# jeongminpark417/COALA-GNN

Measured on AMD Instinct MI355X. Metric: feature-gather GB/s (payload = rows x dim x 4 B delivered per second), IGB-medium GraphSAGE minibatch fetch, higher is better.
Workload: dtype f32

## Files before the change

coala-gnn_amd/COALA_GNN_Pybind/__init__.py:

```python
import ctypes as C
import os
import sys

from . import _capi
from ._capi import CacheConfig, CacheGeometry, CacheProfile, check

_lib = _capi.load()

native = None
if os.path.realpath(_capi.LIB_PATH) == os.path.realpath(os.path.join(os.path.dirname(os.path.abspath(__file__)), os.pardir, "lib", "libcoala_hip.so")):
    try:
        from . import _coala_pybind as native
        if native.abi_version() != _lib.coala_abi_version():
            native = None
    except ImportError:
        native = None

__all__ = [
    "SharedUVAManager", "SSD_GNN_SSD_Controllers", "SSD_GNN_NVSHMEM_Cache", "Isolated_Cache", "Node_distributor_pybind",
    "NVSHMEM_Manager", "Graph_Coloring", "current_stream", "set_stream_provider", "native",
]


def _default_stream_provider():
# ... 150 lines not shown
        if node_distributer is not None:
            color_ptr = node_distributer.get_color_buffer_ptr()
            num_colors = node_distributer.get_num_colors()
            entries = node_distributer.get_num_color_entries()
        if num_rows is None:
            num_rows = entries
        if not num_rows:
            raise RuntimeError("number of feature rows unknown: pass num_rows= or a distributor built with a colour file")
        cfg.num_rows = int(num_rows)
        if color_ptr and entries and entries < cfg.num_rows:
            raise RuntimeError(f"colour table has {entries} entries but the feature table has {cfg.num_rows} rows")
        cfg.node_color = color_ptr
        cfg.num_colors = num_colors
        cfg.max_batch = int(max_batch)
        self._h = C.c_void_p()
        self.dim = ctrls.dim
        self.num_color = num_colors
        self.global_rank = int(g_rank)
        self.local_rank = int(rank)
        self.num_gpus = int(n_gpus)
        check(_lib.coala_cache_create(C.byref(cfg), C.byref(self._h)))
        self._keepalive = node_distributer

    def get_cache_data(self, ret_i_ptr, n_entries=None):
        n = self.num_color if n_entries is None else int(n_entries)
        check(_lib.coala_cache_color_counts(self._h, int(ret_i_ptr), n, current_stream()))

    def get_cache_data_async(self, n_entries=None):
        n = self.num_color if n_entries is None else int(n_entries)
        check(_lib.coala_cache_color_counts_async(self._h, n, current_stream()))

    def get_cache_data_finish(self, ret_i_ptr, n_entries=None):
        n = self.num_color if n_entries is None else int(n_entries)
        check(_lib.coala_cache_color_counts_finish(self._h, int(ret_i_ptr), n))

    def stats(self, reset=False):
        hit, miss, bad = C.c_uint64(), C.c_uint64(), C.c_uint64()
        check(_lib.coala_cache_stats(self._h, C.byref(hit), C.byref(miss), C.byref(bad), int(reset), current_stream()))
        return hit.value, miss.value, bad.value

    def print_stats(self):
        hit, miss, bad = self.stats(reset=True)
        print(f"Global Rank: {self.global_rank} Local Rank:{self.local_rank} hit count: {hit} miss count: {miss}")
        ratio = hit / (hit + miss) if hit + miss else float("nan")
        print(f"Global Rank: {self.global_rank} Local Rank:{self.local_rank}  GPU hit ratio: {ratio:f}")
        if bad:
            print(f"Global Rank: {self.global_rank} Local Rank:{self.local_rank} rejected ids: {bad}")

    def geometry(self):
        g = CacheGeometry()
        check(_lib.coala_cache_geometry(self._h, C.byref(g)))
        return g

    def profile(self, reset=False):
        p = CacheProfile()
        check(_lib.coala_cache_profile(self._h, C.byref(p), int(reset)))
        return p

    def fetch_events(self, enable=True):
        _capi.check(_lib.coala_cache_fetch_events(self._h, 1 if enable else 0))

    def last_fetch_events(self):
        a, b = C.c_void_p(), C.c_void_p()
        _capi.check(_lib.coala_cache_last_fetch_events(self._h, C.byref(a), C.byref(b)))
        return a.value, b.value

    def dump(self):
        import numpy as np
        g = self.geometry()
        keys = np.empty((g.num_sets, 32), dtype=np.uint64)
        cnt = np.empty(g.num_sets, dtype=np.uint32)
        meta = np.empty((g.num_sets, 32), dtype=np.uint32)
        check(_lib.coala_cache_dump(self._h, keys.ctypes.data, cnt.ctypes.data, meta.ctypes.data, current_stream()))
        return keys, cnt, meta

    def close(self):
        if getattr(self, "_h", None):
            _lib.coala_cache_destroy(self._h)
            self._h = C.c_void_p()

    def __del__(self):
        try:
            self.close()
        except Exception:
            pass

    def _read(self, out_ptr, idx_ptr, n):
        if native is not None:
            native.cache_read_feature(self._h.value or 0, int(out_ptr), int(idx_ptr), int(n), current_stream())
        else:
            check(_lib.coala_cache_read_feature(self._h, int(out_ptr), int(idx_ptr), int(n), current_stream()))

    def _serve(self, out_ptr, ids_ptr, n):
        if native is not None:
            native.cache_serve(self._h.value or 0, int(out_ptr), int(ids_ptr), int(n), current_stream())
        else:
            check(_lib.coala_cache_serve(self._h, int(out_ptr), int(ids_ptr), int(n), current_stream()))

    def serve_probe(self, out_ptr, ids_ptr, n):
        check(_lib.coala_cache_serve_probe(self._h, int(out_ptr), int(ids_ptr), int(n), current_stream()))

    def serve_fill(self, out_ptr, ids_ptr, n, begin, end):
        check(_lib.coala_cache_serve_fill(self._h, int(out_ptr), int(ids_ptr), int(n), int(begin), int(end), current_stream()))

    def serve_probe_redirect(self, out_ptr, ids_ptr, n, begin, end, redirect_out_ptr, row_map_ptr=0):
        rd = _capi.RowRedirect(int(begin), int(end), int(redirect_out_ptr) or None, int(row_map_ptr) or None)
# ... 159 lines not shown
```

coala-gnn_amd/COALA_GNN_Pybind/_capi.py:

```python
import ctypes as C
import os

_HERE = os.path.dirname(os.path.abspath(__file__))
LIB_PATH = os.environ.get("COALA_HIP_LIB", os.path.join(os.path.dirname(_HERE), "lib", "libcoala_hip.so"))

OK, EINVAL, EHIP, ENOMEM, EIO, EFORMAT, ERANGE, ECOMM = 0, -1, -2, -3, -4, -5, -6, -7
FLAG_SYNC, FLAG_DISTRIBUTED, FLAG_PROFILE, FLAG_COLD_PARTITIONED, FLAG_TAG64 = 1, 2, 4, 8, 16
WAYS = 32
COUNTS_RING = 8


class CacheConfig(C.Structure):
    _fields_ = [
        ("device", C.c_int32), ("dim", C.c_int32), ("cache_mb", C.c_uint64), ("n_gpus", C.c_int32), ("rank", C.c_int32),
        ("global_rank", C.c_int32), ("flags", C.c_uint32), ("cold_table", C.c_void_p), ("num_rows", C.c_uint64),
        ("node_color", C.c_void_p), ("num_colors", C.c_int32), ("reserved", C.c_int32), ("max_batch", C.c_uint64),
    ]


class CacheGeometry(C.Structure):
    _fields_ = [("num_sets", C.c_uint64), ("num_ways", C.c_uint32), ("cache_dim", C.c_uint32), ("line_bytes", C.c_uint64),
                ("table_bytes", C.c_uint64), ("tag_set_bytes", C.c_uint32), ("reserved", C.c_uint32)]


class CacheProfile(C.Structure):
    _fields_ = [("gather_ms", C.c_double), ("gather_launches", C.c_uint64), ("gather_rows", C.c_uint64),
                ("gather_hits", C.c_uint64), ("fill_ms", C.c_double), ("fill_launches", C.c_uint64),
                ("fill_rows", C.c_uint64), ("event_overhead_us", C.c_double)]


class RowRedirect(C.Structure):
    _fields_ = [("begin", C.c_int64), ("end", C.c_int64), ("out", C.c_void_p), ("row_map", C.c_void_p)]


class SamplerBucketing(C.Structure):
    _fields_ = [("n_parts", C.c_int32), ("reserved", C.c_int32), ("bucketed_nodes", C.c_void_p), ("counts", C.c_void_p),
                ("dst_in_src", C.c_void_p)]


class SamplerLayer(C.Structure):
    _fields_ = [("src_nodes", C.c_void_p), ("nbr_local", C.c_void_p), ("indptr_local", C.c_void_p), ("src_cap", C.c_int64),
                ("edge_cap", C.c_int64)]


class CommProfile(C.Structure):
    _fields_ = [("rows_ms", C.c_double), ("calls", C.c_uint64), ("remote_rows_in", C.c_uint64)]


_VP, _I, _I64, _U64, _SZ = C.c_void_p, C.c_int, C.c_int64, C.c_uint64, C.c_size_t
SYMBOLS = {
    "coala_last_error": (C.c_char_p, []),
    "coala_abi_version": (_I, []),
    "coala_cache_dim": (_I, [_I]),
    "coala_cache_num_sets": (_U64, [_U64, _I]),
    "coala_cache_create": (_I, [C.POINTER(CacheConfig), C.POINTER(_VP)]),
    "coala_cache_destroy": (_I, [_VP]),
    "coala_cache_geometry": (_I, [_VP, C.POINTER(CacheGeometry)]),
    "coala_cache_read_feature": (_I, [_VP, _VP, _VP, _I64, _VP]),
    "coala_cache_serve": (_I, [_VP, _VP, _VP, _I64, _VP]),
    "coala_cache_serve_probe": (_I, [_VP, _VP, _VP, _I64, _VP]),
    "coala_cache_serve_fill": (_I, [_VP, _VP, _VP, _I64, _I64, _I64, _VP]),
    "coala_cache_serve_fill_ranges": (_I, [_VP, _VP, _VP, _I64, C.POINTER(_I64), C.POINTER(_I64), _I, _VP]),
    "coala_cache_serve_abort": (_I, [_VP, _VP]),
    "coala_cache_serve_probe_redirect": (_I, [_VP, _VP, _VP, _I64, C.POINTER(RowRedirect), _VP]),
    "coala_cache_route": (_I, [_VP, _VP, _I64, _I, _I64, _VP, _VP, _VP, _VP, _VP]),
    "coala_cache_scatter": (_I, [_VP, _VP, _VP, _VP, _I64, _VP]),
    "coala_cache_scatter_ranges": (_I, [_VP, _VP, _VP, _VP, C.POINTER(_I64), C.POINTER(_I64), _I, _VP]),
    "coala_cache_row_dim": (_I64, [_VP]),
    "coala_cache_fetch_events": (_I, [_VP, _I]),
    "coala_cache_last_fetch_events": (_I, [_VP, C.POINTER(_VP), C.POINTER(_VP)]),
    "coala_stream_wait_event": (_I, [_VP, _VP]),
    "coala_event_elapsed_ms": (_I, [_VP, _VP, _I, C.POINTER(C.c_float)]),
    "coala_comm_unique_id": (_I, [_VP, _SZ]),
    "coala_comm_create": (_I, [_VP, _I, _I, _I, C.POINTER(_VP)]),
    "coala_comm_destroy": (_I, [_VP]),
    "coala_comm_size": (_I, [_VP]),
    "coala_comm_group_create": (_I, [_I, C.POINTER(_VP)]),
    "coala_comm_group_destroy": (_I, [_VP]),
    "coala_comm_create_inproc": (_I, [_VP, _I, _I, C.POINTER(_VP)]),
    "coala_comm_set_rounds": (_I, [_VP, _I]),
    "coala_comm_get_rounds": (_I, [_VP]),
    "coala_comm_set_self_loopback": (_I, [_VP, _I]),
    "coala_comm_fetch_events": (_I, [_VP, _I]),
    "coala_comm_last_fetch_events": (_I, [_VP, C.POINTER(_VP), C.POINTER(_VP), C.POINTER(_VP)]),
    "coala_comm_profile": (_I, [_VP, _I, C.POINTER(CommProfile), _I]),
    "coala_comm_last_counts": (_I, [_VP, _VP, _VP]),
    "coala_cache_fetch_distributed": (_I, [_VP, _VP, _VP, _VP, _I64, _VP]),
    "coala_cache_fetch_distributed_bucketed": (_I, [_VP, _VP, _VP, _VP, _I64, _VP, _VP]),
    "coala_comm_counts_begin": (_I, [_VP, _VP, _VP, _VP]),
    "coala_cache_fetch_distributed_bucketed_ahead": (_I, [_VP, _VP, _VP, _VP, _I64, _I64, _VP]),
    "coala_cache_color_counts": (_I, [_VP, _VP, C.c_int32, _VP]),
    "coala_cache_color_counts_async": (_I, [_VP, C.c_int32, _VP]),
    "coala_cache_color_counts_finish": (_I, [_VP, _VP, C.c_int32]),
    "coala_cache_stats": (_I, [_VP, C.POINTER(_U64), C.POINTER(_U64), C.POINTER(_U64), _I, _VP]),
    "coala_cache_dump": (_I, [_VP, _VP, _VP, _VP, _VP]),
    "coala_cache_profile": (_I, [_VP, C.POINTER(CacheProfile), _I]),
    "coala_coloring_create": (_I, [_U64, C.POINTER(_VP)]),
    "coala_coloring_destroy": (_I, [_VP]),
    "coala_coloring_set_adj_csc": (_I, [_VP, _VP, _VP]),
    "coala_coloring_set_color_buffer": (_I, [_VP, _VP]),
    "coala_coloring_set_topk_buffers": (_I, [_VP, _VP, _VP, _I]),
    "coala_coloring_color_optimized": (_I, [_VP, _VP, _U64, C.c_uint]),
    "coala_coloring_color_all": (_I, [_VP, C.c_uint]),
    "coala_coloring_num_color": (_U64, [_VP]),
    "coala_coloring_num_color_node": (_U64, [_VP]),
    "coala_coloring_topk": (_I, [_VP, _I]),
    "coala_coloring_nearest": (_I, [_VP]),
    "coala_sampler_create": (_I, [_I, _VP, _VP, _I64, _I64, C.POINTER(_VP)]),
    "coala_sampler_destroy": (_I, [_VP]),
    "coala_sampler_sample": (_I, [_VP, _VP, _I64, C.POINTER(C.c_int32), _I, _U64, _U64, C.POINTER(_VP), C.POINTER(_VP),
# ... 95 lines not shown
```

coala-gnn_amd/csrc/coala_cache.hip:

```cpp
#include <hip/hip_runtime.h>
#include <hip/hip_ext.h>

#include <algorithm>
#include <cstdarg>
#include <cstdio>
#include <cstdlib>
#include <cstring>
#include <new>
#include <type_traits>
#include <utility>
#include <vector>

#include "../../include/coala_hip.h"
#include "coala_internal.h"

namespace {

constexpr uint64_t kEmptyKey = 0xFFFFFFFFFFFFFFFFull;
constexpr uint32_t kLinkMiss = 0x80000000u;
constexpr uint32_t kLinkBad = 0x7FFFFFFFu;
constexpr int kStatBlocks = 2048;
constexpr int kFillSlots = 8;

struct CacheDev {
// ... 236 lines not shown
            const bool h = (G::RPP == 2 && sub) ? h_b : h_a;
            const V* src = reinterpret_cast<const V*>(c.lines + (uint64_t)s * CD);
#pragma unroll
            for (int v = 0; v < G::VPL; ++v) {
                const uint32_t u = v * G::LPR + l_in;
                if (h && (FULL || u < nunits)) val[p][v] = nt_load(src + u);
            }
        }
        if (!SINGLE) {
            tags = load_tags(ids_next);
            ids_next = ids_next2;
        }
#pragma unroll
        for (int p = 0; p < G::PASSES; ++p) {
            const int q = p * G::RPP + sub;
            const bool h_a = row_hit(p * G::RPP), h_b = row_hit(p * G::RPP + (G::RPP - 1));
            const bool bad_a = row_bad(p * G::RPP), bad_b2 = row_bad(p * G::RPP + (G::RPP - 1));
            const bool h = (G::RPP == 2 && sub) ? h_b : h_a;
            const bool bad = (G::RPP == 2 && sub) ? bad_b2 : bad_a;
            V* dst = reinterpret_cast<V*>(out + (base + q) * (int64_t)c.dim);
            if (REDIR) {
                auto row_drow = [&](int r) { return (int32_t)__builtin_amdgcn_readlane(drow_v[r / TG::SPL], TG::LPS * (r % TG::SPL)); };
                const int32_t dr_a = row_drow(p * G::RPP), dr_b = row_drow(p * G::RPP + (G::RPP - 1));
                const int32_t dr = (G::RPP == 2 && sub) ? dr_b : dr_a;
                if (dr >= 0) dst = reinterpret_cast<V*>(rd.out + (int64_t)dr * (int64_t)c.dim);
            }
#pragma unroll
            for (int v = 0; v < G::VPL; ++v) {
                const uint32_t u = v * G::LPR + l_in;
                if (FULL || u < nunits) {
                    if (h) dst[u] = val[p][v];
                    else if (bad) dst[u] = V(0.0f);
                }
            }
        }
#pragma unroll
        for (int t = 0; t < TSTEPS; ++t) {
            if (lead_l[t]) {
                uint32_t w = 0u;
                if (imiss_l[t]) w = kLinkMiss | (((uint32_t)(prev[t] >> 32) == gen) ? (uint32_t)prev[t] : 0u);
                else if (bad_l[t]) w = kLinkBad;
                c.miss_link[base + t * TG::SPL + lane / TG::LPS] = w;
            }
        }
        if (SINGLE) break;
    }
}

__device__ __forceinline__ uint64_t shfl64(uint64_t v, int src) {
    const uint32_t lo = __shfl((int)(uint32_t)v, src), hi = __shfl((int)(uint32_t)(v >> 32), src);
    return ((uint64_t)hi << 32) | lo;
}

template <int CD, int VEC, bool REDIR = false, int NP = 4>
__global__ __launch_bounds__(256) void miss_fill_kernel(CacheDev c, const int64_t* __restrict__ idx, float* __restrict__ out,
                                                        int tile_rows, int sparse_max, uint32_t gen, RangeSet rs, Redirect rd, int dyn_slot) {
    using G = Geo<CD, VEC, NP>;
    using V = typename VecT<VEC>::type;
    constexpr int R = G::R;
    const int lane = threadIdx.x & 63;
    const int64_t wave = (int64_t)blockIdx.x * (blockDim.x >> 6) + (threadIdx.x >> 6);
    const int64_t n_waves = (int64_t)gridDim.x * (blockDim.x >> 6);
    const int64_t n_tiles = ((int64_t)rs.total + tile_rows - 1) / tile_rows;
    const int chunks_per_tile = tile_rows / R;
    const uint32_t nunits = c.dim / VEC;
    const int sub = (G::RPP == 2) ? (lane >> 5) : 0;
    const int l_in = lane & (G::LPR - 1);
    uint32_t my_miss = 0, my_bad = 0;

    constexpr int U = 8;
    uint32_t* ticket = reinterpret_cast<uint32_t*>(c.stats + 2 * kStatBlocks) + (dyn_slot < 0 ? 0 : dyn_slot);
    const bool dyn = dyn_slot >= 0;
    if (reinterpret_cast<const uint32_t*>(c.stats + 2 * kStatBlocks)[2 * kFillSlots + (gen & 1u)] == 0u) return;
    const int64_t n_deal = dyn ? 1 : n_waves;
    const int64_t even8 = n_tiles / (n_waves * 8);
    const int claim_min = even8 < 1 ? 1 : (even8 > U ? U : (int)even8);
    int claim = claim_min;
    for (int64_t unit = dyn ? -1 : wave;;) {
      int64_t claim_end = n_tiles;
      if (dyn) {
          uint32_t t = 0;
          if (lane == 0) t = atomicAdd(ticket, (uint32_t)claim);
          unit = (int64_t)(uint32_t)__builtin_amdgcn_readfirstlane((int)t);
          if (unit >= n_tiles) break;
          claim_end = unit + claim < n_tiles ? unit + claim : n_tiles;
          claim = claim * 2 > 4 * U ? 4 * U : claim * 2;
      } else if (unit >= n_tiles) break;
     for (int64_t tile0 = unit; tile0 < claim_end; tile0 += n_deal * U) {
      const int n_here = dyn ? (int)(claim_end - tile0 < U ? claim_end - tile0 : U) : U;
      uint64_t st_pack = 0;
#pragma unroll
      for (int u = 0; u < U; ++u) {
          const int64_t tile = tile0 + u * n_deal;
          const uint32_t p = (u < n_here && tile < n_tiles && lane < tile_rows) ? pos_of(rs, (uint32_t)(tile * tile_rows + lane)) : 0xFFFFFFFFu;
          const uint32_t w = (p != 0xFFFFFFFFu) ? c.miss_link[p] : 0u;
          const uint64_t v = (w == 0u) ? 0u : ((w & kLinkMiss) ? 1u : 2u);
          st_pack |= v << (8 * u);
      }
      if (!__ballot(st_pack != 0)) continue;
      uint32_t slot_l = 0, win_l = 0;
      uint64_t id_l = 0;
      int64_t drow_l = 0;
      auto rank_at = [&](uint32_t pos) {
          id_l = (uint64_t)idx[pos];
          drow_l = (int64_t)pos;
          if (REDIR && (int64_t)pos >= rd.begin && (int64_t)pos < rd.end)
              drow_l = -((rd.row_map ? rd.row_map[(int64_t)pos - rd.begin] : (int64_t)pos - rd.begin) + 1);
          const uint64_t set = set_of(c, id_l);
          uint32_t cur = (uint32_t)c.set_head[set];
          uint32_t total = 0, rank = 0;
          while (cur) {
              const uint32_t p2 = cur - 1;
              ++total;
              rank += (p2 < pos) ? 1u : 0u;
              cur = c.miss_link[p2] & ~kLinkMiss;
          }
          const uint64_t cv = __hip_atomic_load(c.set_cnt + set, __ATOMIC_RELAXED, __HIP_MEMORY_SCOPE_AGENT);
          const uint32_t cnt0 = ((uint32_t)(cv >> 32) == gen) ? (uint32_t)cv - total : (uint32_t)cv;
          if (rank == 0) __hip_atomic_store(c.set_cnt + set, ((uint64_t)gen << 32) | (uint32_t)(cnt0 + total), __ATOMIC_RELAXED, __HIP_MEMORY_SCOPE_AGENT);
          const uint32_t way = (cnt0 + rank) & (COALA_WAYS - 1);
          slot_l = (uint32_t)(set * COALA_WAYS) + way;
          win_l = (rank + COALA_WAYS >= total) ? 1u : 0u;
          if (win_l) {
              if (c.tag32) reinterpret_cast<uint32_t*>(c.keys)[slot_l] = (uint32_t)id_l;
              else reinterpret_cast<uint64_t*>(c.keys)[slot_l] = id_l;
              if (c.color_counters) {
                  const int32_t col = c.node_color[id_l];
                  atomicSub(c.color_counters + c.color_meta[slot_l], 1);
                  atomicAdd(c.color_counters + col, 1);
                  c.color_meta[slot_l] = (uint32_t)col;
              }
          }
      };
      auto move_group = [&](const int (&srcl)[G::PASSES], const bool (&live)[G::PASSES]) {
          V val[G::PASSES][G::VPL];
          uint32_t slot_[G::PASSES];
          uint64_t id[G::PASSES];
          int64_t drow[G::PASSES];
          bool winner[G::PASSES];
#pragma unroll
          for (int p = 0; p < G::PASSES; ++p) {
              slot_[p] = (uint32_t)__shfl((int)slot_l, srcl[p]);
              winner[p] = __shfl((int)win_l, srcl[p]) != 0;
              id[p] = shfl64(id_l, srcl[p]);
              drow[p] = (int64_t)shfl64((uint64_t)drow_l, srcl[p]);
          }
#pragma unroll
          for (int p = 0; p < G::PASSES; ++p) {
              const V* src = reinterpret_cast<const V*>(c.cold + cold_row_of(c, id[p]) * (uint64_t)c.dim);
#pragma unroll
              for (int v = 0; v < G::VPL; ++v) {
                  const uint32_t u = v * G::LPR + l_in;
                  if (live[p] && u < nunits) val[p][v] = nt_load(src + u);
              }
          }
#pragma unroll
          for (int p = 0; p < G::PASSES; ++p) {
              V* dst = (REDIR && drow[p] < 0) ? reinterpret_cast<V*>(rd.out + (uint64_t)(-(drow[p] + 1)) * c.dim)
                                              : reinterpret_cast<V*>(out + (uint64_t)drow[p] * c.dim);
              V* line = reinterpret_cast<V*>(c.lines + (uint64_t)slot_[p] * CD);
#pragma unroll
              for (int v = 0; v < G::VPL; ++v) {
                  const uint32_t u = v * G::LPR + l_in;
                  if (live[p] && u < nunits) {
                      nt_store(val[p][v], dst + u);
                      if (winner[p]) nt_store(val[p][v], line + u);
                  }
              }
          }
      };
      auto stream_holders = [&](uint64_t holders) {
          int srcl[G::PASSES];
          bool live[G::PASSES];
          while (holders) {
#pragma unroll
              for (int p = 0; p < G::PASSES; ++p) {
                  int l0 = -1, l1 = -1;
                  if (holders) { l0 = __builtin_ctzll(holders); holders &= holders - 1; }
                  if (G::RPP == 2 && holders) { l1 = __builtin_ctzll(holders); holders &= holders - 1; }
                  const int l = (G::RPP == 2 && sub) ? l1 : l0;
                  live[p] = l >= 0;
                  srcl[p] = l >= 0 ? l : 0;
              }
              move_group(srcl, live);
          }
      };
      uint64_t mmask[U];
      uint32_t total_miss = 0, worst = 0;
#pragma unroll
      for (int u = 0; u < U; ++u) {
          const uint8_t st = (uint8_t)(st_pack >> (8 * u));
          mmask[u] = __ballot(st == 1);
          my_miss += (st == 1);
          my_bad += (st == 2);
          const uint32_t cnt = (uint32_t)__builtin_popcountll(mmask[u]);
          total_miss += cnt;
          worst = cnt > worst ? cnt : worst;
      }
      if (!total_miss) continue;
      claim = claim_min;
      if (total_miss <= 64 && (int)worst <= sparse_max) {
          uint32_t k = (uint32_t)lane;
          int u_sel = -1;
          uint64_t m_sel = 0;
#pragma unroll
          for (int u = 0; u < U; ++u) {
              const uint32_t cnt = (uint32_t)__builtin_popcountll(mmask[u]);
              if (u_sel < 0) {
                  if (k < cnt) { u_sel = u; m_sel = mmask[u]; }
                  else k -= cnt;
              }
          }
          if (u_sel >= 0) {
              for (uint32_t i = 0; i < k; ++i) m_sel &= m_sel - 1;
              const uint32_t pos = pos_of(rs, (uint32_t)((tile0 + u_sel * n_deal) * tile_rows + __builtin_ctzll(m_sel)));
              rank_at(pos);
          }
          stream_holders(total_miss >= 64 ? ~0ull : ((1ull << total_miss) - 1ull));
          continue;
      }
#pragma nounroll
      for (int u = 0; u < U; ++u) {
        const uint8_t st = (uint8_t)(st_pack >> (8 * u));
        const uint64_t tile_mask = __ballot(st == 1);
        if (!tile_mask) continue;
        const uint32_t pos_l = st ? pos_of(rs, (uint32_t)((tile0 + u * n_deal) * tile_rows + lane)) : 0u;
        if (__builtin_popcountll(tile_mask) <= sparse_max) {
            if (st == 1) rank_at(pos_l);
            stream_holders(tile_mask);
        } else {
            int srcl[G::PASSES];
            bool live[G::PASSES];
            for (int ck = 0; ck < chunks_per_tile; ++ck) {
                const uint32_t live_mask = (uint32_t)(tile_mask >> (ck * R)) & ((1u << R) - 1u);
                if (!live_mask) continue;
                const int lane0 = ck * R;
                if (st == 1 && lane >= lane0 && lane < lane0 + R) rank_at(pos_l);
#pragma unroll
                for (int p = 0; p < G::PASSES; ++p) {
                    const int q = p * G::RPP + sub;
                    live[p] = (live_mask >> q) & 1;
                    srcl[p] = lane0 + q;
                }
                move_group(srcl, live);
            }
        }
      }
     }
      if (!dyn) break;
    }
    __shared__ uint32_t s_m[256 / 64], s_b[256 / 64];
    for (int off = 32; off > 0; off >>= 1) { my_miss += __shfl_down(my_miss, off); my_bad += __shfl_down(my_bad, off); }
    if (lane == 0) { s_m[threadIdx.x >> 6] = my_miss; s_b[threadIdx.x >> 6] = my_bad; }
    __syncthreads();
    if (threadIdx.x == 0) {
        uint32_t m = 0, b = 0;
        for (int w = 0; w < (int)(blockDim.x >> 6); ++w) { m += s_m[w]; b += s_b[w]; }
        if (m) c.stats[2 * blockIdx.x] += m;
        if (b) c.stats[2 * blockIdx.x + 1] += b;
    }
}

template <int CD, int VEC, int NP = 4>
__global__ __launch_bounds__(256) void scatter_rows_kernel(float* __restrict__ out, const float* __restrict__ src,
                                                           const int64_t* __restrict__ map, RangeSet rs, uint32_t dim) {
    using G = Geo<CD, VEC, NP>;
    using V = typename VecT<VEC>::type;
    constexpr int R = G::R;
    const int lane = threadIdx.x & 63;
    const int64_t wave = (int64_t)blockIdx.x * (blockDim.x >> 6) + (threadIdx.x >> 6);
    const int64_t n_waves = (int64_t)gridDim.x * (blockDim.x >> 6);
    const int64_t n_chunks = ((int64_t)rs.total + R - 1) / R;
    const uint32_t nunits = dim / VEC;
    const int sub = (G::RPP == 2) ? (lane >> 5) : 0;
    const int l_in = lane & (G::LPR - 1);
    for (int64_t chunk = wave; chunk < n_chunks; chunk += n_waves) {
        const int64_t base = chunk * R;
        V val[G::PASSES][G::VPL];
        int64_t d[G::PASSES];
#pragma unroll
        for (int p = 0; p < G::PASSES; ++p) {
            const int64_t vr = base + p * G::RPP + sub;
            const uint32_t r = (vr < (int64_t)rs.total) ? pos_of(rs, (uint32_t)vr) : 0xFFFFFFFFu;
            d[p] = (r != 0xFFFFFFFFu) ? map[r] : -1;
            const V* s = reinterpret_cast<const V*>(src + (int64_t)r * (int64_t)dim);
#pragma unroll
            for (int v = 0; v < G::VPL; ++v) {
                const uint32_t u = v * G::LPR + l_in;
                if (d[p] >= 0 && u < nunits) val[p][v] = nt_load(s + u);
            }
        }
#pragma unroll
        for (int p = 0; p < G::PASSES; ++p) {
            V* t = reinterpret_cast<V*>(out + d[p] * (int64_t)dim);
#pragma unroll
            for (int v = 0; v < G::VPL; ++v) {
                const uint32_t u = v * G::LPR + l_in;
                if (d[p] >= 0 && u < nunits) nt_store(val[p][v], t + u);
            }
        }
    }
}

constexpr int kRouteItems = 4;
constexpr int kRouteTile = 64 * kRouteItems;

__device__ __forceinline__ uint32_t owner_of(uint64_t id, uint32_t n_parts, int pshift) {
    if (pshift >= 0) return (uint32_t)id & (n_parts - 1);
    if ((id >> 32) == 0) return (uint32_t)id % n_parts;
    return (uint32_t)(id % n_parts);
}

__global__ __launch_bounds__(256) void route_count_kernel(const int64_t* __restrict__ idx, int64_t n, uint32_t n_parts,
                                                          int pshift, uint32_t* __restrict__ wave_counts, int64_t n_tiles) {
// ... 40 lines not shown
        for (uint32_t g = 0; g < n_parts; ++g) {
            counts_out[g] = totals[g];
            const int64_t b = bucket_stride > 0 ? (int64_t)g * bucket_stride : acc;
            bases[g] = b;
            if (offsets_out) offsets_out[g] = b;
            acc += totals[g];
        }
        if (offsets_out) offsets_out[n_parts] = bucket_stride > 0 ? (int64_t)n_parts * bucket_stride : acc;
    }
}

__global__ __launch_bounds__(256) void route_scatter_kernel(const int64_t* __restrict__ idx, int64_t n, uint32_t n_parts,
                                                            int pshift, const uint32_t* __restrict__ wave_offsets,
                                                            const int64_t* __restrict__ bases, int64_t* __restrict__ node_out,
                                                            int64_t* __restrict__ map_out, int64_t n_tiles) {
    const int lane = threadIdx.x & 63;
    const int64_t tile = (int64_t)blockIdx.x * (blockDim.x >> 6) + (threadIdx.x >> 6);
    if (tile >= n_tiles) return;
    int64_t off = 0;
    if ((uint32_t)lane < n_parts) off = bases[lane] + (int64_t)wave_offsets[tile * n_parts + lane];
    for (int j = 0; j < kRouteItems; ++j) {
        const int64_t i = tile * kRouteTile + j * 64 + lane;
        const bool valid = i < n;
        const int64_t id = valid ? idx[i] : 0;
        const uint32_t o = valid ? owner_of((uint64_t)id, n_parts, pshift) : 0xFFFFFFFFu;
        int64_t dest = -1;
        for (uint32_t g = 0; g < n_parts; ++g) {
            const uint64_t mask = __ballot(o == g);
            const int64_t bg = __shfl(off, (int)g);
            if (o == g) dest = bg + __builtin_popcountll(mask & ((1ull << lane) - 1ull));
            if ((uint32_t)lane == g) off += __builtin_popcountll(mask);
        }
        if (valid) {
            node_out[dest] = id;
            map_out[dest] = i;
        }
    }
}

}


namespace {

struct LaunchShape {
    int k1_grid_cap;
    int k1_waves;
    bool k1_single;
    int k1_passes;
    int k2_grid_cap;
    int k2_tile_rows;
    int k2_sparse_max;
    int k2_unit_tiles;
};

LaunchShape launch_shape(uint32_t cache_dim, bool host_tier) {
    LaunchShape s;
    s.k1_grid_cap = 16384;
    s.k1_waves = kK1Waves;
    s.k1_single = cache_dim >= 256;
    s.k1_passes = 0;
    const int host_blocks = std::min(64, std::max(24, 16 * 1024 / (int)cache_dim));
    s.k2_grid_cap = host_tier ? host_blocks : kStatBlocks;
    s.k2_tile_rows = host_tier ? 64 : 0;
    s.k2_sparse_max = host_tier ? 32 : 0;
    s.k2_unit_tiles = host_tier ? 1 : 0;
    return s;
}

#ifdef COALA_DEV_KNOBS
void apply_dev_knobs(LaunchShape& s) {
    if (const char* e = getenv("COALA_K1_PASSES")) { int v = atoi(e); if (v == 2 || v == 4 || v == 8 || v == 16) s.k1_passes = v; }
    if (const char* e = getenv("COALA_K1_GRID")) { int g = atoi(e); if (g >= 1 && g <= 65535) s.k1_grid_cap = g; }
    if (const char* e = getenv("COALA_K1_WAVES")) { int w = atoi(e); if (w == 1 || w == 2 || w == 4) s.k1_waves = w; }
    if (const char* e = getenv("COALA_K1_SINGLE")) s.k1_single = atoi(e) != 0;
    if (const char* e = getenv("COALA_K2_TILE_ROWS")) { int t = atoi(e); if (t == 0 || t == 8 || t == 16 || t == 32 || t == 64) s.k2_tile_rows = t; }
    if (const char* e = getenv("COALA_K2_GRID")) { int g = atoi(e); if (g >= 1 && g <= kStatBlocks) s.k2_grid_cap = g; }
    if (const char* e = getenv("COALA_K2_SPARSE")) { int g = atoi(e); if (g >= 0 && g <= 64) s.k2_sparse_max = g; }
    if (const char* e = getenv("COALA_K2_UNIT_TILES")) { int g = atoi(e); if (g >= 0 && g <= 1) s.k2_unit_tiles = g; }
}
#endif

}

struct coala_cache {
    coala_cache_config_t cfg;
    CacheDev d;
    uint64_t cap = 0;
    uint32_t gen = 0;
    int32_t* node_color_dev = nullptr;
    uint32_t* wave_counts = nullptr;
    uint64_t wave_counts_cap = 0;
    int64_t* route_bases = nullptr;
    struct EvPair { hipEvent_t a, b; int kind; uint64_t rows; };
    std::vector<EvPair> ev_live;
    std::vector<hipEvent_t> ev_pool;
    coala_cache_profile_t prof{};
    hipStream_t last_stream = nullptr;
    hipStream_t order_stream = nullptr;
    bool order_set = false;
    hipEvent_t order_ev = nullptr;
    uint64_t table_bytes = 0;
    LaunchShape shape;
    int32_t* color_pin = nullptr;
    int32_t* color_pin_async = nullptr;
    hipEvent_t color_ev = nullptr;
    int32_t color_pending = -1;
    int64_t open_batch_rows = -1;
    std::vector<std::pair<int64_t, int64_t>> open_filled;
    int64_t open_filled_rows = 0;
    Redirect open_redirect{0, 0, nullptr, nullptr};
    int fill_launches = 0;
    uint64_t rows_total = 0;
    uint64_t cum_hit = 0, cum_miss = 0;
    uint64_t prof_hit0 = 0, prof_miss0 = 0;
    bool fetch_events = false;
    static constexpr int kFetchRing = 2048;
    std::vector<hipEvent_t> fev;
    uint64_t fev_calls = 0;
    hipEvent_t last_begin = nullptr, last_end = nullptr;
};

namespace {

#define fail coala_fail_
#define HIPCHK COALA_HIPCHK

int follow_stream(coala_cache* h, hipStream_t s) {
    if (h->order_set && h->order_stream != s) {
        if (!h->order_ev) HIPCHK(hipEventCreateWithFlags(&h->order_ev, hipEventDisableTiming));
        if (hipEventRecord(h->order_ev, h->order_stream) == hipSuccess) HIPCHK(hipStreamWaitEvent(s, h->order_ev, 0));
        else (void)hipGetLastError();
// ... 245 lines not shown
    delete h;
    return COALA_OK;
}

int64_t coala_cache_row_dim(const coala_cache_t* h) { return h ? (int64_t)h->d.dim : 0; }

int coala_cache_fetch_events(coala_cache_t* h, int enable) {
    if (!h) return fail(COALA_EINVAL, "null handle");
    h->fetch_events = enable != 0;
    if (!h->fetch_events) h->last_begin = h->last_end = nullptr;
    return COALA_OK;
}

int coala_cache_last_fetch_events(const coala_cache_t* h, void** begin_ev, void** end_ev) {
    if (!h) return fail(COALA_EINVAL, "null handle");
    if (begin_ev) *begin_ev = (void*)h->last_begin;
    if (end_ev) *end_ev = (void*)h->last_end;
    return COALA_OK;
}

int coala_stream_wait_event(void* stream, void* event) {
    if (!event) return fail(COALA_EINVAL, "null event");
    HIPCHK(hipStreamWaitEvent((hipStream_t)stream, (hipEvent_t)event, 0));
    return COALA_OK;
}

int coala_event_elapsed_ms(void* begin_ev, void* end_ev, int wait, float* ms_out) {
    if (!begin_ev || !end_ev || !ms_out) return fail(COALA_EINVAL, "null argument");
    if (wait) HIPCHK(hipEventSynchronize((hipEvent_t)end_ev));
    else {
        const hipError_t q = hipEventQuery((hipEvent_t)end_ev);
        if (q == hipErrorNotReady) {
            (void)hipGetLastError();
            return 1;
        }
        if (q != hipSuccess) return fail(COALA_EHIP, "hipEventQuery failed: %s", hipGetErrorString(q));
    }
    HIPCHK(hipEventElapsedTime(ms_out, (hipEvent_t)begin_ev, (hipEvent_t)end_ev));
    return COALA_OK;
}

int coala_cache_geometry(const coala_cache_t* h, coala_cache_geometry_t* out) {
    if (!h || !out) return fail(COALA_EINVAL, "null argument");
    out->num_sets = h->d.num_sets;
    out->num_ways = COALA_WAYS;
    out->cache_dim = h->d.cache_dim;
    out->line_bytes = (uint64_t)h->d.cache_dim * 4;
    out->table_bytes = h->table_bytes;
    out->tag_set_bytes = h->d.tag32 ? COALA_WAYS * 4u : COALA_WAYS * 8u;
    out->reserved = 0;
    return COALA_OK;
}

enum { kPhaseProbe = 1, kPhaseFill = 2, kPhaseBoth = 3 };

static int read_feature_impl(coala_cache_t* h, float* out, const int64_t* idx, int64_t n, void* stream, bool force_dist,
                             int phases, const int64_t* begins, const int64_t* ends, int n_ranges,
                             const coala_row_redirect_t* redirect, hipEvent_t ext_begin = nullptr, hipEvent_t ext_end = nullptr,
                             hipEvent_t* rode = nullptr) {
    if (rode) rode[0] = rode[1] = nullptr;
    if (!h) return fail(COALA_EINVAL, "null handle");
    h->last_begin = h->last_end = nullptr;
    if (n < 0 || n > 0x7FFFFFFFll) return fail(COALA_EINVAL, "n=%lld out of range", (long long)n);
    if (phases & kPhaseProbe) {
        if (h->open_batch_rows >= 0)
            return fail(COALA_EINVAL, "a batch of %lld rows is still open (%lld filled): finish its serve_fill calls or call coala_cache_serve_abort",
                        (long long)h->open_batch_rows, (long long)h->open_filled_rows);
    } else if (h->open_batch_rows != n || h->gen == 0) {
        return fail(COALA_EINVAL, "serve_fill without a matching serve_probe (batch of %lld rows, probe saw %lld)", (long long)n, (long long)h->open_batch_rows);
    }
    if (n == 0) return COALA_OK;
    if (!idx || (!out && !(redirect && redirect->begin == 0 && redirect->end == n))) return fail(COALA_EINVAL, "null buffer");
    Redirect rd{0, 0, nullptr, nullptr};
    if (phases & kPhaseProbe) {
        if (redirect && redirect->end > redirect->begin) {
            if (redirect->begin < 0 || redirect->end > n || !redirect->out)
                return fail(COALA_EINVAL, "redirect [%lld, %lld) outside the batch of %lld rows, or null destination", (long long)redirect->begin, (long long)redirect->end, (long long)n);
            rd = Redirect{redirect->begin, redirect->end, redirect->out, redirect->row_map};
        }
    } else {
        rd = h->open_redirect;
    }
    const int64_t whole_b = 0, whole_e = n;
    if (phases == kPhaseBoth) { begins = &whole_b; ends = &whole_e; n_ranges = 1; }
    int64_t fill_rows = 0;
    if (phases & kPhaseFill) {
        if (n_ranges < 0 || (n_ranges > 0 && (!begins || !ends))) return fail(COALA_EINVAL, "bad fill ranges");
        std::vector<std::pair<int64_t, int64_t>> add;
        for (int k = 0; k < n_ranges; ++k) {
            if (begins[k] < 0 || begins[k] > ends[k] || ends[k] > n)
                return fail(COALA_EINVAL, "fill range [%lld, %lld) outside the batch of %lld rows", (long long)begins[k], (long long)ends[k], (long long)n);
            if (ends[k] > begins[k]) add.emplace_back(begins[k], ends[k]);
        }
        if (phases == kPhaseFill) {
            std::vector<std::pair<int64_t, int64_t>> all = h->open_filled;
            all.insert(all.end(), add.begin(), add.end());
            std::sort(all.begin(), all.end());
            for (size_t k = 1; k < all.size(); ++k)
                if (all[k].first < all[k - 1].second)
                    return fail(COALA_EINVAL, "fill range [%lld, %lld) overlaps positions that were already filled in this batch", (long long)all[k].first, (long long)all[k].second);
            h->open_filled.swap(all);
        }
        for (auto& r : add) fill_rows += r.second - r.first;
        if (fill_rows == 0 && !(phases & kPhaseProbe)) return COALA_OK;
    }
    hipStream_t s = (hipStream_t)stream;
// ... 44 lines not shown
        constexpr int CD = geo_cd(geo);
        constexpr int VEC = geo_vec(geo);
        using G = Geo<CD, VEC>;
        if (phases & kPhaseProbe) {
            ProfScope ps(h, s, 0, (uint64_t)n, fe_begin, nullptr);
            if (rode) rode[0] = ps.on ? ps.a : fe_begin;
            const bool full = (VEC == 4) && ((int)d.dim == CD);
            auto launch_k1 = [&](auto tag_c, auto np_c) {
                using TAG = decltype(tag_c);
                constexpr int NP = decltype(np_c)::value;
                constexpr int NPR = (Geo<CD, VEC, NP>::R > 8) ? NP / 2 : NP;
                using GK = Geo<CD, VEC, NP>;
                using GR = Geo<CD, VEC, NPR>;
                const int64_t chunks = redir ? (n + GR::R - 1) / GR::R : (n + GK::R - 1) / GK::R;
                const LaunchShape& ls = h->shape;
                const bool single = ls.k1_single && chunks <= kK1SingleMaxChunks;
                const dim3 grid(grid_for(chunks, ls.k1_waves, single ? (int)((kK1SingleMaxChunks + ls.k1_waves - 1) / ls.k1_waves) : ls.k1_grid_cap)), block(64 * ls.k1_waves);
                auto pick = [&](auto single_c) {
                    constexpr bool S = decltype(single_c)::value;
                    if (redir) return full ? probe_gather_kernel<CD, VEC, TAG, NPR, true, true, S> : probe_gather_kernel<CD, VEC, TAG, NPR, false, true, S>;
                    return full ? probe_gather_kernel<CD, VEC, TAG, NP, true, false, S> : probe_gather_kernel<CD, VEC, TAG, NP, false, false, S>;
                };
                ps.launch(single ? pick(std::true_type{}) : pick(std::false_type{}), grid, block, idx, out, n, gen, (uint32_t)grid.x, d, rd);
            };
#ifdef COALA_DEV_KNOBS
            if (h->shape.k1_passes) {
                auto by_np = [&](auto tag_c) {
                    switch (h->shape.k1_passes) {
                        case 2: launch_k1(tag_c, std::integral_constant<int, 2>{}); break;
                        case 8: launch_k1(tag_c, std::integral_constant<int, 8>{}); break;
                        case 16: launch_k1(tag_c, std::integral_constant<int, (Geo<CD, VEC, 16>::R <= 32 ? 16 : 8)>{}); break;
                        default: launch_k1(tag_c, std::integral_constant<int, 4>{}); break;
                    }
                };
                if (d.tag32) by_np(uint32_t{}); else by_np(uint64_t{});
            } else
#endif
            if (d.tag32) launch_k1(uint32_t{}, std::integral_constant<int, kK1Passes>{});
            else launch_k1(uint64_t{}, std::integral_constant<int, kK1Passes>{});
        }
        if ((phases & kPhaseFill) && fill_rows > 0) {
            const int tile_rows = h->shape.k2_tile_rows > 0 ? h->shape.k2_tile_rows : G::R;
            return for_each_range_set(begins, ends, n_ranges, [&](const RangeSet& rs) -> int {
                const bool last_set = ++set_no == n_sets;
                ProfScope ps(h, s, 2, 0, nullptr, last_set ? fe_end : nullptr);
                if (rode && last_set) rode[1] = ps.on ? ps.b : fe_end;
                const int64_t tiles = ((int64_t)rs.total + tile_rows - 1) / tile_rows;
                const dim3 grid(grid_for(tiles, 4, h->shape.k2_grid_cap));
                const int64_t waves = (int64_t)grid.x * 4;
                int dyn_slot = -1;
                if (h->shape.k2_unit_tiles > 0 && tiles > waves && tiles < 0x7FFFFFFF && h->fill_launches < kFillSlots)
                    dyn_slot = (int)((gen & 1u) * kFillSlots) + h->fill_launches;
                h->fill_launches++;
                if (redir) ps.launch(miss_fill_kernel<CD, VEC, true>, grid, dim3(256), d, idx, out, tile_rows, h->shape.k2_sparse_max, gen, rs, rd, dyn_slot);
                else ps.launch(miss_fill_kernel<CD, VEC, false>, grid, dim3(256), d, idx, out, tile_rows, h->shape.k2_sparse_max, gen, rs, rd, dyn_slot);
                return COALA_OK;
            });
        }
        return COALA_OK;
    });
    if (rc) return rc;
    if (own_ring) {
        h->last_begin = fe_begin;
        h->last_end = fe_end;
        h->fev_calls++;
    }
    if (phases & kPhaseProbe) h->rows_total += (uint64_t)n;
    if (phases == kPhaseFill) {
        h->open_filled_rows += fill_rows;
        if (h->open_filled_rows == h->open_batch_rows) {
            h->open_batch_rows = -1;
            h->open_filled.clear();
            h->open_filled_rows = 0;
        }
    }
    HIPCHK(hipGetLastError());
    if (h->cfg.flags & COALA_FLAG_SYNC) HIPCHK(hipStreamSynchronize(s));
    return COALA_OK;
}

int coala_cache_read_feature(coala_cache_t* h, float* out, const int64_t* idx, int64_t n, void* stream) {
    return read_feature_impl(h, out, idx, n, stream, false, kPhaseBoth, nullptr, nullptr, 0, nullptr);
}

int coala_cache_serve(coala_cache_t* h, float* out, const int64_t* ids, int64_t n, void* stream) {
    return read_feature_impl(h, out, ids, n, stream, true, kPhaseBoth, nullptr, nullptr, 0, nullptr);
}

int coala_cache_serve_probe(coala_cache_t* h, float* out, const int64_t* ids, int64_t n, void* stream) {
    return read_feature_impl(h, out, ids, n, stream, true, kPhaseProbe, nullptr, nullptr, 0, nullptr);
}

int coala_cache_serve_probe_redirect(coala_cache_t* h, float* out, const int64_t* ids, int64_t n, const coala_row_redirect_t* redirect,
                                     void* stream) {
    return read_feature_impl(h, out, ids, n, stream, true, kPhaseProbe, nullptr, nullptr, 0, redirect);
}

int coala_serve_probe_redirect_ev_(coala_cache_t* h, float* out, const int64_t* ids, int64_t n, const coala_row_redirect_t* redirect, void* stream,
                                   hipEvent_t begin_ev, hipEvent_t* rode) {
    hipEvent_t r[2];
    const int rc = read_feature_impl(h, out, ids, n, stream, true, kPhaseProbe, nullptr, nullptr, 0, redirect, begin_ev, nullptr, r);
    if (rode) *rode = r[0];
    return rc;
}
int coala_serve_fill_ranges_ev_(coala_cache_t* h, float* out, const int64_t* ids, int64_t n, const int64_t* begins, const int64_t* ends, int n_ranges,
                                void* stream, hipEvent_t end_ev, hipEvent_t* rode) {
    hipEvent_t r[2];
    const int rc = read_feature_impl(h, out, ids, n, stream, true, kPhaseFill, begins, ends, n_ranges, nullptr, nullptr, end_ev, r);
// ... 221 lines not shown
```

include/coala_hip.h:

```cpp
#ifndef COALA_HIP_H
#define COALA_HIP_H

#include <stddef.h>
#include <stdint.h>

#ifdef __cplusplus
extern "C" {
#endif

#define COALA_OK 0
#define COALA_EINVAL (-1)
#define COALA_EHIP (-2)
#define COALA_ENOMEM (-3)
#define COALA_EIO (-4)
#define COALA_EFORMAT (-5)
#define COALA_ERANGE (-6)
#define COALA_ECOMM (-7)

#define COALA_WAYS 32u
#define COALA_COUNTS_RING 8

#define COALA_FLAG_SYNC 1u
#define COALA_FLAG_DISTRIBUTED 2u
#define COALA_FLAG_PROFILE 4u
#define COALA_FLAG_TAG64 16u
#define COALA_FLAG_COLD_PARTITIONED 8u

const char* coala_last_error(void);
int coala_abi_version(void);

int coala_cache_dim(int dim);
uint64_t coala_cache_num_sets(uint64_t cache_mb, int cache_dim);

typedef struct coala_cache coala_cache_t;

typedef struct coala_cache_config {
    int32_t device;
    int32_t dim;
    uint64_t cache_mb;
    int32_t n_gpus;
    int32_t rank;
    int32_t global_rank;
    uint32_t flags;
    const float* cold_table;
    uint64_t num_rows;
    const int64_t* node_color;
    int32_t num_colors;
    int32_t reserved;
    uint64_t max_batch;
} coala_cache_config_t;

int coala_cache_create(const coala_cache_config_t* cfg, coala_cache_t** out);
int coala_cache_destroy(coala_cache_t* h);

typedef struct coala_cache_geometry {
    uint64_t num_sets;
    uint32_t num_ways;
    uint32_t cache_dim;
    uint64_t line_bytes;
    uint64_t table_bytes;
    uint32_t tag_set_bytes;
    uint32_t reserved;
} coala_cache_geometry_t;
int coala_cache_geometry(const coala_cache_t* h, coala_cache_geometry_t* out);

int coala_cache_read_feature(coala_cache_t* h, float* out, const int64_t* idx, int64_t n, void* stream);

int coala_cache_serve(coala_cache_t* h, float* out, const int64_t* ids, int64_t n, void* stream);

int coala_cache_serve_probe(coala_cache_t* h, float* out, const int64_t* ids, int64_t n, void* stream);
int coala_cache_serve_fill(coala_cache_t* h, float* out, const int64_t* ids, int64_t n, int64_t begin, int64_t end, void* stream);
int coala_cache_serve_fill_ranges(coala_cache_t* h, float* out, const int64_t* ids, int64_t n, const int64_t* begins,
                                  const int64_t* ends, int n_ranges, void* stream);
int coala_cache_serve_abort(coala_cache_t* h, void* stream);

typedef struct coala_row_redirect {
    int64_t begin, end;
    float* out;
    const int64_t* row_map;
} coala_row_redirect_t;
int coala_cache_serve_probe_redirect(coala_cache_t* h, float* out, const int64_t* ids, int64_t n, const coala_row_redirect_t* redirect,
                                     void* stream);

int coala_cache_route(coala_cache_t* h, const int64_t* idx, int64_t n, int n_parts, int64_t bucket_stride,
                      int64_t* node_out, int64_t* map_out, int64_t* counts_out, int64_t* offsets_out, void* stream);

int coala_cache_scatter(coala_cache_t* h, float* out, const float* src, const int64_t* map, int64_t n, void* stream);
int coala_cache_scatter_ranges(coala_cache_t* h, float* out, const float* src, const int64_t* map, const int64_t* begins,
                               const int64_t* ends, int n_ranges, void* stream);

int64_t coala_cache_row_dim(const coala_cache_t* h);

typedef struct coala_comm coala_comm_t;
int coala_comm_unique_id(void* out_id, size_t cap);
int coala_comm_create(const void* id_bytes, int rank, int nranks, int device, coala_comm_t** out);
int coala_comm_destroy(coala_comm_t* c);
int coala_comm_size(const coala_comm_t* c);
typedef struct coala_comm_group coala_comm_group_t;
int coala_comm_group_create(int nranks, coala_comm_group_t** out);
int coala_comm_group_destroy(coala_comm_group_t* g);
int coala_comm_create_inproc(coala_comm_group_t* g, int rank, int device, coala_comm_t** out);
int coala_comm_set_rounds(coala_comm_t* c, int rounds);
int coala_comm_get_rounds(const coala_comm_t* c);
int coala_comm_set_self_loopback(coala_comm_t* c, int on);
int coala_comm_last_counts(const coala_comm_t* c, int64_t* send, int64_t* recv);
int coala_cache_fetch_distributed(coala_cache_t* h, coala_comm_t* c, float* out, const int64_t* idx, int64_t n, void* stream);
int coala_cache_fetch_distributed_bucketed(coala_cache_t* h, coala_comm_t* c, float* out, const int64_t* idx, int64_t n,
                                           const int64_t* counts_dev, void* stream);
int coala_comm_counts_begin(coala_comm_t* c, const int64_t* counts_dev, void* stream, int64_t* ticket_out);
int coala_cache_fetch_distributed_bucketed_ahead(coala_cache_t* h, coala_comm_t* c, float* out, const int64_t* idx, int64_t n,
                                                 int64_t ticket, void* stream);
int coala_cache_fetch_events(coala_cache_t* h, int enable);
int coala_cache_last_fetch_events(const coala_cache_t* h, void** begin_ev, void** end_ev);
int coala_stream_wait_event(void* stream, void* event);
int coala_event_elapsed_ms(void* begin_ev, void* end_ev, int wait, float* ms_out);

int coala_comm_fetch_events(coala_comm_t* c, int enable);
// ... 195 lines not shown
```

Baseline: 81.65.

## Double-buffer cold-row loads in miss-fill kernel for host-tier caches

Adds a PIPE variant of the miss-fill kernel that splits row movement into issue and drain phases and keeps two groups of cold-row loads in flight. This lets host-memory reads overlap with the stores of the previous group and with the set-rank lookup. Group size is picked from a register budget. For host-tier caches it also halves the tile rows and the sparse threshold and turns the pipeline on by default. The kernel gains register pressure and some dummy loads for dead lanes, and a fill-shape query API is added.

```diff
diff --git a/coala-gnn_amd/COALA_GNN_Pybind/__init__.py b/coala-gnn_amd/COALA_GNN_Pybind/__init__.py
--- a/coala-gnn_amd/COALA_GNN_Pybind/__init__.py
+++ b/coala-gnn_amd/COALA_GNN_Pybind/__init__.py
@@ -226,6 +226,11 @@
         check(_lib.coala_cache_geometry(self._h, C.byref(g)))
         return g
 
+    def fill_shape(self, aligned16=True):
+        v = [C.c_int() for _ in range(4)]
+        check(_lib.coala_cache_fill_shape(self._h, 1 if aligned16 else 0, *[C.byref(x) for x in v]))
+        return tuple(x.value for x in v)
+
     def profile(self, reset=False):
         p = CacheProfile()
         check(_lib.coala_cache_profile(self._h, C.byref(p), int(reset)))
diff --git a/coala-gnn_amd/COALA_GNN_Pybind/_capi.py b/coala-gnn_amd/COALA_GNN_Pybind/_capi.py
--- a/coala-gnn_amd/COALA_GNN_Pybind/_capi.py
+++ b/coala-gnn_amd/COALA_GNN_Pybind/_capi.py
@@ -56,6 +56,7 @@
     "coala_cache_create": (_I, [C.POINTER(CacheConfig), C.POINTER(_VP)]),
     "coala_cache_destroy": (_I, [_VP]),
     "coala_cache_geometry": (_I, [_VP, C.POINTER(CacheGeometry)]),
+    "coala_cache_fill_shape": (_I, [_VP, _I, C.POINTER(_I), C.POINTER(_I), C.POINTER(_I), C.POINTER(_I)]),
     "coala_cache_read_feature": (_I, [_VP, _VP, _VP, _I64, _VP]),
     "coala_cache_serve": (_I, [_VP, _VP, _VP, _I64, _VP]),
     "coala_cache_serve_probe": (_I, [_VP, _VP, _VP, _I64, _VP]),
diff --git a/coala-gnn_amd/csrc/coala_cache.hip b/coala-gnn_amd/csrc/coala_cache.hip
--- a/coala-gnn_amd/csrc/coala_cache.hip
+++ b/coala-gnn_amd/csrc/coala_cache.hip
@@ -312,12 +312,13 @@
     return ((uint64_t)hi << 32) | lo;
 }
 
-template <int CD, int VEC, bool REDIR = false, int NP = 4>
+template <int CD, int VEC, bool REDIR = false, int NP = 4, bool PIPE = false>
 __global__ __launch_bounds__(256) void miss_fill_kernel(CacheDev c, const int64_t* __restrict__ idx, float* __restrict__ out,
                                                         int tile_rows, int sparse_max, uint32_t gen, RangeSet rs, Redirect rd, int dyn_slot) {
     using G = Geo<CD, VEC, NP>;
     using V = typename VecT<VEC>::type;
     constexpr int R = G::R;
+    static_assert(R <= 32, "per-chunk row masks are 32 bits wide");
     const int lane = threadIdx.x & 63;
     const int64_t wave = (int64_t)blockIdx.x * (blockDim.x >> 6) + (threadIdx.x >> 6);
     const int64_t n_waves = (int64_t)gridDim.x * (blockDim.x >> 6);
@@ -361,11 +362,14 @@
       uint32_t slot_l = 0, win_l = 0;
       uint64_t id_l = 0;
       int64_t drow_l = 0;
-      auto rank_at = [&](uint32_t pos) {
+      auto head_at = [&](uint32_t pos) {
           id_l = (uint64_t)idx[pos];
           drow_l = (int64_t)pos;
           if (REDIR && (int64_t)pos >= rd.begin && (int64_t)pos < rd.end)
               drow_l = -((rd.row_map ? rd.row_map[(int64_t)pos - rd.begin] : (int64_t)pos - rd.begin) + 1);
+      };
+      auto rank_at = [&](uint32_t pos) {
+          if (!PIPE) head_at(pos);
           const uint64_t set = set_of(c, id_l);
           uint32_t cur = (uint32_t)c.set_head[set];
           uint32_t total = 0, rank = 0;
@@ -392,27 +396,33 @@
               }
           }
       };
-      auto move_group = [&](const int (&srcl)[G::PASSES], const bool (&live)[G::PASSES]) {
-          V val[G::PASSES][G::VPL];
+      struct Grp { int srcl[G::PASSES]; bool live[G::PASSES]; };
+      auto issue_group = [&](const Grp& g, V (&val)[G::PASSES][G::VPL]) {
+          uint64_t id[G::PASSES];
+#pragma unroll
+          for (int p = 0; p < G::PASSES; ++p) id[p] = shfl64(id_l, g.srcl[p]);
+#pragma unroll
+          for (int p = 0; p < G::PASSES; ++p) {
+              const V* src = reinterpret_cast<const V*>(c.cold + cold_row_of(c, id[p]) * (uint64_t)c.dim);
+#pragma unroll
+              for (int v = 0; v < G::VPL; ++v) {
+                  const uint32_t u = v * G::LPR + l_in;
+                  if (PIPE) {
+                      const bool on = g.live[p] && u < nunits;
+                      val[p][v] = nt_load(on ? src + u : reinterpret_cast<const V*>(c.lines));
+                  } else if (g.live[p] && u < nunits) val[p][v] = nt_load(src + u);
+              }
+          }
+      };
+      auto drain_group = [&](const Grp& g, const V (&val)[G::PASSES][G::VPL]) {
           uint32_t slot_[G::PASSES];
-          uint64_t id[G::PASSES];
           int64_t drow[G::PASSES];
           bool winner[G::PASSES];
 #pragma unroll
           for (int p = 0; p < G::PASSES; ++p) {
-              slot_[p] = (uint32_t)__shfl((int)slot_l, srcl[p]);
-              winner[p] = __shfl((int)win_l, srcl[p]) != 0;
-              id[p] = shfl64(id_l, srcl[p]);
-              drow[p] = (int64_t)shfl64((uint64_t)drow_l, srcl[p]);
-          }
-#pragma unroll
-          for (int p = 0; p < G::PASSES; ++p) {
-              const V* src = reinterpret_cast<const V*>(c.cold + cold_row_of(c, id[p]) * (uint64_t)c.dim);
-#pragma unroll
-              for (int v = 0; v < G::VPL; ++v) {
-                  const uint32_t u = v * G::LPR + l_in;
-                  if (live[p] && u < nunits) val[p][v] = nt_load(src + u);
-              }
+              slot_[p] = (uint32_t)__shfl((int)slot_l, g.srcl[p]);
+              winner[p] = __shfl((int)win_l, g.srcl[p]) != 0;
+              drow[p] = (int64_t)shfl64((uint64_t)drow_l, g.srcl[p]);
           }
 #pragma unroll
           for (int p = 0; p < G::PASSES; ++p) {
@@ -422,27 +432,71 @@
 #pragma unroll
               for (int v = 0; v < G::VPL; ++v) {
                   const uint32_t u = v * G::LPR + l_in;
-                  if (live[p] && u < nunits) {
+                  if (g.live[p] && u < nunits) {
                       nt_store(val[p][v], dst + u);
                       if (winner[p]) nt_store(val[p][v], line + u);
                   }
               }
           }
       };
+      auto group_of = [&](uint64_t gm) {
+          Grp g;
+#pragma unroll
+          for (int p = 0; p < G::PASSES; ++p) {
+              int l0 = -1, l1 = -1;
+              if (gm) { l0 = __builtin_ctzll(gm); gm &= gm - 1; }
+              if (G::RPP == 2 && gm) { l1 = __builtin_ctzll(gm); gm &= gm - 1; }
+              const int l = (G::RPP == 2 && sub) ? l1 : l0;
+              g.live[p] = l >= 0;
+              g.srcl[p] = l >= 0 ? l : 0;
+          }
+          return g;
+      };
       auto stream_holders = [&](uint64_t holders) {
-          int srcl[G::PASSES];
-          bool live[G::PASSES];
           while (holders) {
-#pragma unroll
-              for (int p = 0; p < G::PASSES; ++p) {
-                  int l0 = -1, l1 = -1;
-                  if (holders) { l0 = __builtin_ctzll(holders); holders &= holders - 1; }
-                  if (G::RPP == 2 && holders) { l1 = __builtin_ctzll(holders); holders &= holders - 1; }
-                  const int l = (G::RPP == 2 && sub) ? l1 : l0;
-                  live[p] = l >= 0;
-                  srcl[p] = l >= 0 ? l : 0;
+              uint64_t gm = 0;
+#pragma unroll
+              for (int q = 0; q < R; ++q)
+                  if (holders) { gm |= holders & (0 - holders); holders &= holders - 1; }
+              const Grp g = group_of(gm);
+              V val[G::PASSES][G::VPL];
+              issue_group(g, val);
+              drain_group(g, val);
+          }
+      };
+      auto pipe_stream = [&](uint64_t holders, bool dense, bool mine, uint32_t pos_h) {
+          auto take = [&]() {
+              uint64_t gm = 0;
+              if (dense) {
+                  if (holders) gm = holders & (((1ull << R) - 1ull) << ((__builtin_ctzll(holders) / R) * R));
+              } else {
+                  uint64_t h = holders;
+#pragma unroll
+                  for (int q = 0; q < R; ++q)
+                      if (h) { gm |= h & (0 - h); h &= h - 1; }
               }
-              move_group(srcl, live);
+              holders &= ~gm;
+              return gm;
+          };
+          if (mine) head_at(pos_h);
+          V buf_a[G::PASSES][G::VPL], buf_b[G::PASSES][G::VPL];
+          Grp ga = group_of(take()), gb = ga;
+          issue_group(ga, buf_a);
+          uint64_t m = take();
+          bool hb = m != 0;
+          if (hb) { gb = group_of(m); issue_group(gb, buf_b); }
+          if (mine) rank_at(pos_h);
+          for (;;) {
+              drain_group(ga, buf_a);
+              m = take();
+              const bool ha = m != 0;
+              if (ha) { ga = group_of(m); issue_group(ga, buf_a); }
+              if (!hb) break;
+              drain_group(gb, buf_b);
+              m = take();
+              hb = m != 0;
+              if (hb) { gb = group_of(m); issue_group(gb, buf_b); }
+              if (!ha) break;
           }
       };
       uint64_t mmask[U];
@@ -471,12 +525,15 @@
                   else k -= cnt;
               }
           }
+          uint32_t pos_sel = 0;
           if (u_sel >= 0) {
               for (uint32_t i = 0; i < k; ++i) m_sel &= m_sel - 1;
-              const uint32_t pos = pos_of(rs, (uint32_t)((tile0 + u_sel * n_deal) * tile_rows + __builtin_ctzll(m_sel)));
-              rank_at(pos);
+              pos_sel = pos_of(rs, (uint32_t)((tile0 + u_sel * n_deal) * tile_rows + __builtin_ctzll(m_sel)));
+              if (!PIPE) rank_at(pos_sel);
           }
-          stream_holders(total_miss >= 64 ? ~0ull : ((1ull << total_miss) - 1ull));
+          const uint64_t holders = total_miss >= 64 ? ~0ull : ((1ull << total_miss) - 1ull);
+          if (PIPE) pipe_stream(holders, false, u_sel >= 0, pos_sel);
+          else stream_holders(holders);
           continue;
       }
 #pragma nounroll
@@ -485,12 +542,13 @@
         const uint64_t tile_mask = __ballot(st == 1);
         if (!tile_mask) continue;
         const uint32_t pos_l = st ? pos_of(rs, (uint32_t)((tile0 + u * n_deal) * tile_rows + lane)) : 0u;
-        if (__builtin_popcountll(tile_mask) <= sparse_max) {
+        if (PIPE) {
+            pipe_stream(tile_mask, __builtin_popcountll(tile_mask) > sparse_max, st == 1, pos_l);
+        } else if (__builtin_popcountll(tile_mask) <= sparse_max) {
             if (st == 1) rank_at(pos_l);
             stream_holders(tile_mask);
         } else {
-            int srcl[G::PASSES];
-            bool live[G::PASSES];
+            Grp g;
             for (int ck = 0; ck < chunks_per_tile; ++ck) {
                 const uint32_t live_mask = (uint32_t)(tile_mask >> (ck * R)) & ((1u << R) - 1u);
                 if (!live_mask) continue;
@@ -499,10 +557,12 @@
 #pragma unroll
                 for (int p = 0; p < G::PASSES; ++p) {
                     const int q = p * G::RPP + sub;
-                    live[p] = (live_mask >> q) & 1;
-                    srcl[p] = lane0 + q;
+                    g.live[p] = (live_mask >> q) & 1;
+                    g.srcl[p] = lane0 + q;
                 }
-                move_group(srcl, live);
+                V val[G::PASSES][G::VPL];
+                issue_group(g, val);
+                drain_group(g, val);
             }
         }
       }
@@ -520,6 +580,15 @@
         if (b) c.stats[2 * blockIdx.x + 1] += b;
     }
 }
+
+constexpr int kK2PipeRegs = 64;
+template <int CD, int VEC> struct K2Pipe {
+    using G1 = Geo<CD, VEC, 1>;
+    static constexpr int kPerPass = G1::VPL * VEC;
+    static constexpr int kFit = kK2PipeRegs / kPerPass < 1 ? 1 : kK2PipeRegs / kPerPass;
+    static constexpr int NP = kFit > 16 ? 16 : kFit;
+    static_assert(64 % Geo<CD, VEC, NP>::R == 0, "a verdict tile is a whole number of groups");
+};
 
 template <int CD, int VEC, int NP = 4>
 __global__ __launch_bounds__(256) void scatter_rows_kernel(float* __restrict__ out, const float* __restrict__ src,
@@ -666,6 +735,7 @@
     int k2_tile_rows;
     int k2_sparse_max;
     int k2_unit_tiles;
+    bool k2_pipe;
 };
 
 LaunchShape launch_shape(uint32_t cache_dim, bool host_tier) {
@@ -676,9 +746,10 @@
     s.k1_passes = 0;
     const int host_blocks = std::min(64, std::max(24, 16 * 1024 / (int)cache_dim));
     s.k2_grid_cap = host_tier ? host_blocks : kStatBlocks;
-    s.k2_tile_rows = host_tier ? 64 : 0;
-    s.k2_sparse_max = host_tier ? 32 : 0;
+    s.k2_tile_rows = host_tier ? 32 : 0;
+    s.k2_sparse_max = host_tier ? 16 : 0;
     s.k2_unit_tiles = host_tier ? 1 : 0;
+    s.k2_pipe = host_tier;
     return s;
 }
 
@@ -692,6 +763,8 @@
     if (const char* e = getenv("COALA_K2_GRID")) { int g = atoi(e); if (g >= 1 && g <= kStatBlocks) s.k2_grid_cap = g; }
     if (const char* e = getenv("COALA_K2_SPARSE")) { int g = atoi(e); if (g >= 0 && g <= 64) s.k2_sparse_max = g; }
     if (const char* e = getenv("COALA_K2_UNIT_TILES")) { int g = atoi(e); if (g >= 0 && g <= 1) s.k2_unit_tiles = g; }
+    if (const char* e = getenv("COALA_K2_PIPE")) s.k2_pipe = atoi(e) != 0;
+    if (s.k2_tile_rows == 0) s.k2_pipe = false;
 }
 #endif
 
@@ -1043,6 +1116,20 @@
     return COALA_OK;
 }
 
+int coala_cache_fill_shape(const coala_cache_t* h, int aligned16, int* group_rows, int* groups_in_flight, int* tile_rows, int* sparse_max) {
+    if (!h || !group_rows || !groups_in_flight || !tile_rows || !sparse_max) return fail(COALA_EINVAL, "null argument");
+    const bool pipe = h->shape.k2_pipe;
+    return dispatch_geo(h->d.cache_dim, aligned16 != 0, [&](auto geo) -> int {
+        constexpr int CD = geo_cd(geo);
+        constexpr int VEC = geo_vec(geo);
+        *group_rows = pipe ? Geo<CD, VEC, K2Pipe<CD, VEC>::NP>::R : Geo<CD, VEC>::R;
+        *groups_in_flight = pipe ? 2 : 1;
+        *tile_rows = h->shape.k2_tile_rows > 0 ? h->shape.k2_tile_rows : Geo<CD, VEC>::R;
+        *sparse_max = h->shape.k2_sparse_max;
+        return COALA_OK;
+    });
+}
+
 enum { kPhaseProbe = 1, kPhaseFill = 2, kPhaseBoth = 3 };
 
 static int read_feature_impl(coala_cache_t* h, float* out, const int64_t* idx, int64_t n, void* stream, bool force_dist,
@@ -1193,8 +1280,12 @@
                 if (h->shape.k2_unit_tiles > 0 && tiles > waves && tiles < 0x7FFFFFFF && h->fill_launches < kFillSlots)
                     dyn_slot = (int)((gen & 1u) * kFillSlots) + h->fill_launches;
                 h->fill_launches++;
-                if (redir) ps.launch(miss_fill_kernel<CD, VEC, true>, grid, dim3(256), d, idx, out, tile_rows, h->shape.k2_sparse_max, gen, rs, rd, dyn_slot);
-                else ps.launch(miss_fill_kernel<CD, VEC, false>, grid, dim3(256), d, idx, out, tile_rows, h->shape.k2_sparse_max, gen, rs, rd, dyn_slot);
+                constexpr int NPP = K2Pipe<CD, VEC>::NP;
+                constexpr int NPR = (Geo<CD, VEC, NPP>::R > 16) ? NPP / 2 : NPP;
+                auto k2 = h->shape.k2_pipe
+                              ? (redir ? miss_fill_kernel<CD, VEC, true, NPR, true> : miss_fill_kernel<CD, VEC, false, NPP, true>)
+                              : (redir ? miss_fill_kernel<CD, VEC, true> : miss_fill_kernel<CD, VEC, false>);
+                ps.launch(k2, grid, dim3(256), d, idx, out, tile_rows, h->shape.k2_sparse_max, gen, rs, rd, dyn_slot);
                 return COALA_OK;
             });
         }
diff --git a/include/coala_hip.h b/include/coala_hip.h
--- a/include/coala_hip.h
+++ b/include/coala_hip.h
@@ -63,6 +63,7 @@
     uint32_t reserved;
 } coala_cache_geometry_t;
 int coala_cache_geometry(const coala_cache_t* h, coala_cache_geometry_t* out);
+int coala_cache_fill_shape(const coala_cache_t* h, int aligned16, int* group_rows, int* groups_in_flight, int* tile_rows, int* sparse_max);
 
 int coala_cache_read_feature(coala_cache_t* h, float* out, const int64_t* idx, int64_t n, void* stream);
 
```

New measurement: 82.18 (median of 6 runs). No clear change (+0.6%).
